# zkp-gravity/0g-halo2

Measured on AMD Instinct MI355X. Metric: create_proof proofs/hour, model_28input_256entry_1hash_1bpi, higher is better.
Workload: dtype u32x8 (254-bit Montgomery integers)

## Files before the change

### 0g-halo2_amd/csrc/field.h

```cpp
#pragma once

#include <hip/hip_runtime.h>
#include <stdint.h>

#define ZG_HD __host__ __device__ __forceinline__

namespace zg {

struct alignas(16) Fe {
    uint32_t l[8];
};

struct FrParams {
    static ZG_HD uint32_t p(int i) {
        constexpr uint32_t P[8] = {0xf0000001u, 0x43e1f593u, 0x79b97091u, 0x2833e848u,
                                   0x8181585du, 0xb85045b6u, 0xe131a029u, 0x30644e72u};
        return P[i];
    }
    static constexpr uint32_t P_TOP = 0x30644e72u;
    static constexpr uint32_t INV = 0xefffffffu;
    static constexpr bool IS_FR = true;
    static ZG_HD Fe one() {
        return Fe{{0x4ffffffbu, 0xac96341cu, 0x9f60cd29u, 0x36fc7695u, 0x7879462eu, 0x666ea36fu,
                   0x9a07df2fu, 0x0e0a77c1u}};
// ... 129 lines not shown
#include "mont_mul_gfx950.inc"
        Fe o;
#pragma unroll
        for (int i = 0; i < 8; i++) o.l[i] = r[i];
        reduce_once(o);
        return o;
#else
        typedef unsigned __int128 u128;
        uint64_t A[4], B[4], M[4], t[6] = {0, 0, 0, 0, 0, 0};
        for (int i = 0; i < 4; i++) {
            A[i] = (uint64_t)a.l[2 * i] | ((uint64_t)a.l[2 * i + 1] << 32);
            B[i] = (uint64_t)b.l[2 * i] | ((uint64_t)b.l[2 * i + 1] << 32);
            M[i] = (uint64_t)P::p(2 * i) | ((uint64_t)P::p(2 * i + 1) << 32);
        }
        const uint64_t ninv32 = P::INV;
        const uint64_t inv64 = ninv32 * (2 + M[0] * ninv32);
        for (int i = 0; i < 4; i++) {
            u128 c = 0;
            for (int j = 0; j < 4; j++) {
                c += (u128)A[j] * B[i] + t[j];
                t[j] = (uint64_t)c;
                c >>= 64;
            }
            c += t[4];
            t[4] = (uint64_t)c;
            t[5] = (uint64_t)(c >> 64);
            const uint64_t m = t[0] * inv64;
            c = (u128)m * M[0] + t[0];
            c >>= 64;
            for (int j = 1; j < 4; j++) {
                c += (u128)m * M[j] + t[j];
                t[j - 1] = (uint64_t)c;
                c >>= 64;
            }
            c += t[4];
            t[3] = (uint64_t)c;
            t[4] = t[5] + (uint64_t)(c >> 64);
        }
        Fe o;
        for (int i = 0; i < 4; i++) {
            o.l[2 * i] = (uint32_t)t[i];
            o.l[2 * i + 1] = (uint32_t)(t[i] >> 32);
        }
        reduce_once(o);
        return o;
#endif
    }

    static ZG_HD Fe sqr(const Fe& a) { return mul(a, a); }

    static ZG_HD Fe from_raw(const Fe& a) { return mul(a, P::r2()); }

    static ZG_HD Fe to_raw(const Fe& a) {
        Fe one_raw = fe_zero();
        one_raw.l[0] = 1;
        return mul(a, one_raw);
    }

    static ZG_HD Fe from_u64(uint64_t v) {
        Fe t = fe_zero();
        t.l[0] = (uint32_t)v;
        t.l[1] = (uint32_t)(v >> 32);
        return from_raw(t);
    }

    static ZG_HD Fe pow(const Fe& a, const uint32_t e[8]) {
        Fe res = one();
        for (int i = 7; i >= 0; i--)
            for (int b = 31; b >= 0; b--) {
                res = sqr(res);
                if ((e[i] >> b) & 1) res = mul(res, a);
            }
        return res;
    }

    static ZG_HD Fe pow_u64(const Fe& a, uint64_t e) {
        Fe res = one();
        bool started = false;
        for (int b = 63; b >= 0; b--) {
            if (started) res = sqr(res);
            if ((e >> b) & 1) {
                res = mul(res, a);
                started = true;
            }
        }
        return res;
    }

    static ZG_HD Fe inv_fermat(const Fe& a) {
        uint32_t e[8];
#pragma unroll
        for (int i = 0; i < 8; i++) e[i] = P::p(i);
        e[0] -= 2;
        return pow(a, e);
    }

    static ZG_HD Fe inv(const Fe& a) {
        if (fe_is_zero(a)) return a;
#if !defined(__HIP_DEVICE_COMPILE__)
        {
            typedef unsigned __int128 u128;
            uint64_t pm4[4], u[4], v[4], x1[4] = {1, 0, 0, 0}, x2[4] = {0, 0, 0, 0};
            for (int i = 0; i < 4; i++) {
                pm4[i] = (uint64_t)P::p(2 * i) | ((uint64_t)P::p(2 * i + 1) << 32);
                u[i] = (uint64_t)a.l[2 * i] | ((uint64_t)a.l[2 * i + 1] << 32);
                v[i] = pm4[i];
            }
            auto add4 = [](uint64_t* o, const uint64_t* x, const uint64_t* y) {
                u128 c = 0;
// ... 138 lines not shown
```

### 0g-halo2_amd/csrc/msm.hip

```cpp
#include <cstdlib>

#include "msm.h"
#include "field9.h"

namespace zg {

constexpr uint32_t MSM_K_THROUGHPUT = 48, MSM_K_LATENCY = 16;
constexpr uint32_t MSM_MAX_C = 16;
constexpr uint32_t MSM_LEN_BINS = 128;
constexpr uint32_t MSM_HEAVY = 16;
constexpr uint32_t MSM_HEAVY_THROUGHPUT = 4;
constexpr uint32_t MSM_AFFINE_ROUNDS = 0;
constexpr uint32_t MSM_MAX_BATCH = 4096;

__device__ __forceinline__ Fe ld_fe_g(const Fe* p) {
    Fe r;
    const uint4* q = reinterpret_cast<const uint4*>(p);
    uint4 a = q[0], b = q[1];
    r.l[0] = a.x; r.l[1] = a.y; r.l[2] = a.z; r.l[3] = a.w;
    r.l[4] = b.x; r.l[5] = b.y; r.l[6] = b.z; r.l[7] = b.w;
    return r;
}
__device__ __forceinline__ void st_fe_g(Fe* p, const Fe& v) {
    uint4* q = reinterpret_cast<uint4*>(p);
    q[0] = make_uint4(v.l[0], v.l[1], v.l[2], v.l[3]);
    q[1] = make_uint4(v.l[4], v.l[5], v.l[6], v.l[7]);
}
__device__ __forceinline__ XYZZ ld_xyzz(const XYZZ* p) {
    XYZZ r;
    r.x = ld_fe_g(&p->x); r.y = ld_fe_g(&p->y); r.zz = ld_fe_g(&p->zz); r.zzz = ld_fe_g(&p->zzz);
    return r;
}
__device__ __forceinline__ void st_xyzz(XYZZ* p, const XYZZ& v) {
    st_fe_g(&p->x, v.x); st_fe_g(&p->y, v.y); st_fe_g(&p->zz, v.zz); st_fe_g(&p->zzz, v.zzz);
}

__global__ void msm_table_kernel(const Affine* __restrict__ bases, Affine* __restrict__ table,
                                 uint32_t n, uint32_t c, uint32_t windows) {
    uint32_t i = blockIdx.x * blockDim.x + threadIdx.x;
    if (i >= n) return;
    const Fe c261 = Fq9Params::c261_fe();
    Affine p;
    p.x = ld_fe_g(&bases[i].x);
    p.y = ld_fe_g(&bases[i].y);
    st_fe_g(&table[i].x, Fq::mul(p.x, c261));
    st_fe_g(&table[i].y, Fq::mul(p.y, c261));
    for (uint32_t w = 1; w < windows; w++) {
        XYZZ acc = xyzz_dbl_affine(p);
        for (uint32_t d = 1; d < c; d++) acc = xyzz_dbl(acc);
        p = xyzz_to_affine(acc);
        st_fe_g(&table[(size_t)w * n + i].x, Fq::mul(p.x, c261));
        st_fe_g(&table[(size_t)w * n + i].y, Fq::mul(p.y, c261));
    }
}

__global__ __launch_bounds__(256) void msm_digits_kernel(const Fe* __restrict__ scalars, size_t stride, uint32_t per,
                                                         size_t outer, uint32_t n,
                                                         uint32_t c, uint32_t windows, uint32_t tbits,
                                                         uint32_t* __restrict__ dig, uint64_t run_mask) {
    uint32_t i = blockIdx.x * blockDim.x + threadIdx.x, b = blockIdx.y;
    if (i >= n) return;
    const uint32_t nb = 1u << (c - 1);
    const uint32_t j = b % per;
    const Fe* sv = scalars + (size_t)(b / per) * outer + (size_t)j * stride;
    Fe s = ld_fe_g(sv + i);
    uint32_t flip = 0;
    if (j < 64 && ((run_mask >> j) & 1ull)) {
        if (i + 1 < n) s = Fr::sub(s, ld_fe_g(sv + i + 1));
        s = Fr::to_raw(s);
        Fe neg;
        uint32_t ps[8], pr[8];
#pragma unroll
        for (int j = 0; j < 8; j++) {
            ps[j] = s.l[j];
            pr[j] = FrParams::p(j);
        }
        uint32_t nl[8];
        sub8(nl, pr, ps);
#pragma unroll
        for (int j = 0; j < 8; j++) neg.l[j] = nl[j];
        bool smaller = false;
        for (int j = 7; j >= 0; j--) {
            if (neg.l[j] != s.l[j]) {
                smaller = neg.l[j] < s.l[j];
                break;
            }
        }
        if (smaller && !fe_is_zero(s)) {
            s = neg;
            flip = 1u << 31;
        }
    } else {
        s = Fr::to_raw(s);
    }
    uint32_t l[9];
#pragma unroll
    for (int j = 0; j < 8; j++) l[j] = s.l[j];
    l[8] = 0;
    const uint32_t top_lo = c * (windows - 1) - 1;
    bool large = false;
#pragma unroll
    for (int j = 0; j < 8; j++) {
        const uint32_t lo_bit = 32u * j;
        if (lo_bit + 32 > top_lo) {
            uint32_t v = l[j];
            if (lo_bit < top_lo) v >>= (top_lo - lo_bit);
            large |= v != 0;
        }
    }
    if (large && tbits) {
        const uint32_t t = ((l[0] >> 5) ^ (l[1] >> 11) ^ l[2]) & ((1u << tbits) - 1);
        uint64_t carry = 0;
#pragma unroll
        for (int j = 0; j < 8; j++) {
            carry += (uint64_t)l[j] + (uint64_t)t * FrParams::p(j);
            l[j] = (uint32_t)carry;
            carry >>= 32;
        }
        l[8] = (uint32_t)carry;
    }
    uint64_t bits = (uint64_t)l[0] | ((uint64_t)l[1] << 32);
    uint32_t have = 64, next = 2, carry = 0;
    uint32_t* db = dig + (size_t)b * windows * n + i;
    for (uint32_t w = 0; w < windows; w++) {
        if (have < c && next < 9) {
            uint32_t limb = next == 2 ? l[2] : next == 3 ? l[3] : next == 4 ? l[4] : next == 5 ? l[5]
                          : next == 6 ? l[6] : next == 7 ? l[7] : l[8];
            bits |= (uint64_t)limb << have;
            have += 32;
            next++;
        }
        uint32_t d = (uint32_t)(bits & ((1u << c) - 1)) + carry;
        bits >>= c;
        have = have >= c ? have - c : 0;
        carry = d > nb ? 1u : 0u;
        uint32_t k = carry ? (1u << c) - d : d;
        db[(size_t)w * n] = k ? (k | ((carry << 31) ^ flip)) : 0u;
    }
}

static_assert((FrParams::P_TOP >> 30) == 0, "msm_digits_naf_kernel: the scalar field's modulus must be below 2^254");
__global__ __launch_bounds__(256) void msm_digits_naf_kernel(const Fe* __restrict__ scalars, size_t stride, uint32_t per,
                                                             size_t outer, uint32_t n, uint32_t w, uint32_t slots,
                                                             uint32_t* __restrict__ dig, uint64_t run_mask, uint32_t balanced) {
    const uint32_t i = blockIdx.x * blockDim.x + threadIdx.x, b = blockIdx.y;
    if (i >= n) return;
    const uint32_t vj = b % per;
    const Fe* sv = scalars + (size_t)(b / per) * outer + (size_t)vj * stride;
    Fe s = ld_fe_g(sv + i);
    uint32_t flip = 0;
    if (vj < 64 && ((run_mask >> vj) & 1ull)) {
        if (i + 1 < n) s = Fr::sub(s, ld_fe_g(sv + i + 1));
        s = Fr::to_raw(s);
        Fe neg, pr;
#pragma unroll
        for (int j = 0; j < 8; j++) pr.l[j] = FrParams::p(j);
        sub8(neg.l, pr.l, s.l);
        bool smaller = false;
        for (int j = 7; j >= 0; j--) {
            if (neg.l[j] != s.l[j]) {
                smaller = neg.l[j] < s.l[j];
                break;
            }
        }
        if (smaller && !fe_is_zero(s)) {
            s = neg;
            flip = 0x80000000u;
        }
    } else {
        s = Fr::to_raw(s);
    }
    uint64_t bits = (uint64_t)s.l[0];
    uint32_t have = 32, next = 1, pos = 0, slot = 0;
    uint32_t* db = dig + (size_t)b * slots * n + i;
    const uint32_t mask = (1u << w) - 1u, half = 1u << (w - 1);
    for (;;) {
        if (have <= 16 && next < 8) {
            const uint32_t limb = next == 1 ? s.l[1] : next == 2 ? s.l[2] : next == 3 ? s.l[3] : next == 4 ? s.l[4]
                                : next == 5 ? s.l[5] : next == 6 ? s.l[6] : s.l[7];
            bits += (uint64_t)limb << have;
            have += 32;
            next++;
        }
        if (bits == 0 && next >= 8) break;
        if ((bits & 1ull) == 0) {
            uint32_t z = bits ? (uint32_t)__ffsll((long long)bits) - 1u : have;
            if (z > have) z = have;
            if (z == 0) z = 1;
            bits >>= z;
            have -= z;
            pos += z;
            continue;
        }
        uint32_t wd = w, m = mask, hf = half;
        if (balanced && next >= 8) {
            const uint32_t rem = 64u - (uint32_t)__clzll((long long)bits);
            if (rem <= w - 1u) {
                if (slot < slots && pos <= 254u) db[(size_t)slot * n] = (((uint32_t)bits + 1u) >> 1) | (pos << 16) | flip;
                slot++;
                break;
            }
            if (rem <= 2u * (w - 1u)) {
                wd = (rem + 1u) >> 1;
                m = (1u << wd) - 1u;
                hf = 1u << (wd - 1u);
            }
        }
        const uint32_t v = (uint32_t)bits & m;
        const bool neg = v > hf;
        const uint32_t d = neg ? (m + 1u) - v : v;
        if (slot < slots && pos <= 254u) db[(size_t)slot * n] = ((d + 1u) >> 1) | (pos << 16) | ((neg ? 0x80000000u : 0u) ^ flip);
        slot++;
        bits = (bits >> wd) + (neg ? 1ull : 0ull);
        have = have >= wd ? have - wd : 0;
        pos += wd;
    }
    for (; slot < slots; slot++) db[(size_t)slot * n] = 0u;
}

__global__ __launch_bounds__(1024) void msm_hist_kernel(const uint32_t* __restrict__ dig, uint32_t n, uint32_t c,
                                                        uint32_t windows, uint32_t* __restrict__ cnt,
// ... 668 lines not shown
template <int L, uint32_t RB>
__global__ __launch_bounds__(L * RB) void msm_bucket_sum_kernel(const XYZZ9* __restrict__ sfx,
                                                                                   const XYZZ9* __restrict__ blk_p,
                                                                                   XYZZ9* __restrict__ blk_w,
                                                                                   uint32_t nblk, uint32_t* __restrict__ tickets,
                                                                                   XYZZ* __restrict__ out, uint32_t odd,
                                                                                   XYZZ9* __restrict__ tsum) {
    __shared__ XYZZ9 sh[RB];
    __shared__ XYZZ9 bs;
    const uint32_t j = threadIdx.x / L, role = threadIdx.x % L;
    const uint32_t blk = blockIdx.x, b = blockIdx.y;
    if (role == 0) sh[j] = blk + 1 + j < nblk ? ld_xyzz9(blk_p + (size_t)b * nblk + blk + 1 + j) : xyzz9_identity();
    __syncthreads();
    uint32_t span = 1;
    while (span < nblk) span <<= 1;
    auto tree_step = [&](uint32_t o) {
        if (j < o) xstore<true>(&sh[j], xaddl<L>(&sh[j], &sh[j + o], role));
        __syncthreads();
    };
    for (uint32_t o = span / 2; o > 0; o >>= 1) tree_step(o);
    if (threadIdx.x == 0) bs = sh[0];
    __syncthreads();
    xstore<true>(&sh[j], xaddl<L>(sfx + ((size_t)b * nblk + blk) * RB + j, &bs, role));
    __syncthreads();
    if (odd && blk == 0 && threadIdx.x == 0) st_xyzz9(tsum + b, sh[0]);
    __syncthreads();
    for (uint32_t o = RB / 2; o > 0; o >>= 1) tree_step(o);
    __shared__ uint32_t ticket;
    if (threadIdx.x == 0) {
        st_xyzz9(blk_w + (size_t)b * nblk + blk, sh[0]);
        __threadfence();
        ticket = atomicAdd(tickets + b, 1u);
    }
    __syncthreads();
    if (ticket != nblk - 1) return;
    __threadfence();
    if (role == 0) sh[j] = j < nblk ? ld_xyzz9(blk_w + (size_t)b * nblk + j) : xyzz9_identity();
    __syncthreads();
    for (uint32_t o = span / 2; o > 0; o >>= 1) tree_step(o);
    if (threadIdx.x == 0) {
        XYZZ9 R = sh[0];
        if (odd) {
            XYZZ9 T = ld_xyzz9(tsum + b);
            R = xyzz9_add(R, R);
            T.y = f9_neg(T.y);
            R = xyzz9_add(R, T);
        }
        st_xyzz(out + b, xyzz9_to_xyzz(R, false));
        tickets[b] = 0;
    }
}

constexpr uint32_t MSM_STRIP = 8;
constexpr uint32_t MSM_STRIP_LANES = 256;

__global__ __launch_bounds__(256) void msm_strip_kernel(const XYZZ9* __restrict__ partial, const uint32_t* __restrict__ toff,
                                                        const uint32_t* __restrict__ hmap, const XYZZ9* __restrict__ hsum,
                                                        uint32_t max_tasks, uint32_t max_heavy, uint32_t c, uint32_t nstrips,
                                                        XYZZ9* __restrict__ strip_u, XYZZ9* __restrict__ strip_loc, uint32_t S) {
    const uint32_t j = blockIdx.x * blockDim.x + threadIdx.x, b = blockIdx.y;
    if (j >= nstrips) return;
    const uint32_t nb = 1u << (c - 1);
    const uint32_t* to = toff + (size_t)b * (nb + 2);
    const XYZZ9* pp = partial + (size_t)b * max_tasks;
    XYZZ9 run = xyzz9_identity(), loc = xyzz9_identity();
    for (uint32_t s = S; s-- > 0;) {
        const uint32_t k = j * S + s + 1;
        if (k <= nb) {
            const uint32_t hs = hmap[(size_t)b * (nb + 1) + k];
            if (hs < max_heavy) {
                run = xyzz9_add(run, ld_xyzz9(hsum + (size_t)b * max_heavy + hs));
            } else {
                const uint32_t t0 = to[k], t1 = to[k + 1];
                for (uint32_t t = t0; t < t1; t++) run = xyzz9_add(run, ld_xyzz9(pp + t));
            }
        }
        loc = xyzz9_add(loc, run);
    }
    st_xyzz9(strip_u + (size_t)b * nstrips + j, run);
    st_xyzz9(strip_loc + (size_t)b * nstrips + j, loc);
}

__global__ __launch_bounds__(MSM_STRIP_LANES) void msm_strip_sum_kernel(const XYZZ9* __restrict__ strip_u,
                                                                       const XYZZ9* __restrict__ strip_loc, uint32_t nstrips,
                                                                       uint32_t per, XYZZ* __restrict__ out, uint32_t S, uint32_t odd) {
    __shared__ XYZZ9 sh[MSM_STRIP_LANES];
    const uint32_t l = threadIdx.x, b = blockIdx.x;
    const XYZZ9* U = strip_u + (size_t)b * nstrips;
    const XYZZ9* L = strip_loc + (size_t)b * nstrips;
    XYZZ9 C = xyzz9_identity(), w = xyzz9_identity(), a = xyzz9_identity();
    for (uint32_t t = per; t-- > 0;) {
        const uint32_t jj = l * per + t;
        if (jj >= nstrips) continue;
        w = xyzz9_add(w, C);
        C = xyzz9_add(C, ld_xyzz9(U + jj));
        a = xyzz9_add(a, ld_xyzz9(L + jj));
    }
    auto tree = [&](XYZZ9 v) {
        sh[l] = v;
        __syncthreads();
        for (uint32_t o = MSM_STRIP_LANES / 2; o > 0; o >>= 1) {
            if (l < o) sh[l] = xyzz9_add(sh[l], sh[l + o]);
            __syncthreads();
        }
        XYZZ9 r = sh[0];
        __syncthreads();
        return r;
    };
    sh[l] = C;
    __syncthreads();
    for (uint32_t o = 1; o < MSM_STRIP_LANES; o <<= 1) {
        XYZZ9 v = xyzz9_identity();
        const bool has = l + o < MSM_STRIP_LANES;
        if (has) v = sh[l + o];
        __syncthreads();
        if (has) sh[l] = xyzz9_add(sh[l], v);
        __syncthreads();
    }
    XYZZ9 sfx = l >= 1 ? sh[l] : xyzz9_identity();
    __syncthreads();
    XYZZ9 X = sfx;
    for (uint32_t d = per; d > 1; d >>= 1) X = xyzz9_dbl(X);
    X = xyzz9_add(X, w);
    for (uint32_t d = S; d > 1; d >>= 1) X = xyzz9_dbl(X);
    XYZZ9 Y = xyzz9_add(X, a);
    if (odd) {
        Y = xyzz9_dbl(Y);
        XYZZ9 nc = C;
        nc.y = f9_neg(nc.y);
        Y = xyzz9_add(Y, nc);
    }
    const XYZZ9 R = tree(Y);
    if (l != 0) return;
    st_xyzz(out + b, xyzz9_to_xyzz(R, false));
}

static uint32_t default_window_bits(size_t n) {
    if (const int v = knob(K_MSM_C); v >= 2 && v <= (int)MSM_MAX_C) return (uint32_t)v;
    uint32_t lg = 0;
    while (((size_t)1 << (lg + 1)) <= n) lg++;
    int c = lg >= 14 ? (int)lg - 2 : (int)lg - 1;
    if (c < 4) c = 4;
    if (c > (int)MSM_MAX_C) c = MSM_MAX_C;
    return (uint32_t)c;
}

int bases_register_dev(zg_ctx* ctx, const Affine* d_bases, size_t n, uint32_t window_bits, zg_bases** out) {
    ZG_REQUIRE(n > 0 && n < (1u << 23), ZG_ERR_UNSUPPORTED, "zg_bases_register: n=%zu out of range", n);
    uint32_t c = window_bits ? window_bits : default_window_bits(n);
    ZG_REQUIRE(c >= 1 && c <= MSM_MAX_C, ZG_ERR_INVALID_ARG, "zg_bases_register: window_bits %u not in [2,16]", c);
    uint32_t windows = (255 + c - 1) / c;
    zg_bases* b = new zg_bases();
    b->ctx = ctx;
    b->device = ctx->device;
    b->n = n;
    b->c = c;
    b->windows = windows;
    hipError_t e = hipMalloc(&b->table, (size_t)windows * n * sizeof(Affine));
    if (e != hipSuccess) {
        set_error("zg_bases_register: hipMalloc(%zu) failed: %s", (size_t)windows * n * sizeof(Affine),
                  hipGetErrorString(e));
        delete b;
        return ZG_ERR_OOM;
    }
    hipLaunchKernelGGL(msm_table_kernel, dim3((uint32_t)((n + 63) / 64)), dim3(64), 0, ctx->stream, d_bases,
                       b->table, (uint32_t)n, c, windows);
// ... 475 lines not shown
    uint32_t R;
    size_t cap;
    uint64_t left;
    uint32_t max_tasks;
    bool pair_tasks;
    uint32_t rb, nblk;
    int lanes;
    uint32_t heavy_thr, max_heavy;
    uint32_t strip, nstrips, strip_per;
    uint32_t tbits;
    uint32_t topsplit;
};
static int msm_plan(const zg_ctx* ctx, const MsmJob& j, uint32_t naf, MsmPlan* out) {
    MsmPlan p{};
    const size_t n = j.n;
    p.B = (uint32_t)j.batch; p.N = (uint32_t)n; p.naf = naf;
    p.c = naf ? naf - 1 : j.bases->c; p.W = naf ? 254 / naf + 1 : j.bases->windows; p.nb = 1u << (p.c - 1);
    const int k_env = knob(K_MSM_K);
    const int kl_env = knob(K_MSM_K_LAT);
    const uint32_t k_lat_default = n >= (1u << 17) ? 48u : n >= (1u << 16) ? 32u : MSM_K_LATENCY;
    p.K = ctx->msm_pair ? (kl_env >= 4 && kl_env <= 120 ? (uint32_t)kl_env : k_lat_default)
                        : (k_env >= 4 && k_env <= 120 ? (uint32_t)k_env : MSM_K_THROUGHPUT);
    p.entries = (uint64_t)p.N * p.W;
    ZG_REQUIRE(p.entries < (1ull << 31), ZG_ERR_UNSUPPORTED, "zg_msm: n*windows too large");
    const int aff_env = knob(K_MSM_AFFINE);
    p.R = ctx->msm_pair ? 0u : aff_env >= 0 && aff_env <= 4 ? (uint32_t)aff_env : MSM_AFFINE_ROUNDS;
    const uint64_t padm = (1ull << p.R) - 1ull;
    p.cap = (size_t)((p.entries + (uint64_t)p.nb * padm + padm) & ~padm);
    ZG_REQUIRE(p.cap < (1ull << 31), ZG_ERR_UNSUPPORTED, "zg_msm: n*windows too large");
    p.left = p.cap >> p.R;
    p.max_tasks = (uint32_t)(p.left / p.K + (p.left < p.nb ? p.left : p.nb) + 1);
    p.pair_tasks = ctx->msm_pair && p.N < (1u << 16);
    p.rb = MSM_RB;
    p.lanes = 1;
    if (ctx->msm_pair) {
        const int rb_env = knob(K_MSM_RB), lanes_env = knob(K_MSM_LANES);
        const uint32_t nblk64 = (p.nb + 63) / 64;
        const bool quad_fits = nblk64 <= 64 && (uint64_t)nblk64 * p.B <= (uint64_t)ctx->num_cus;
        uint32_t want = rb_env == 64 || rb_env == 128 || rb_env == 256 ? (uint32_t)rb_env : quad_fits ? 64u : 128u;
        if ((p.nb + want - 1) / want <= want) p.rb = want;
        p.lanes = lanes_env == 2 || lanes_env == 4 ? lanes_env : p.rb == 64 ? 4 : 2;
        if (p.rb > 128) p.lanes = 2;
    }
    p.nblk = (p.nb + p.rb - 1) / p.rb;
    ZG_REQUIRE(p.nblk <= 256 && p.nblk <= p.rb, ZG_ERR_UNSUPPORTED, "zg_msm: window_bits %u too large", p.c);
    const int hv_env = knob(K_MSM_HEAVY);
    p.heavy_thr = hv_env >= 1 && hv_env <= 64 ? (uint32_t)hv_env : ctx->msm_pair ? MSM_HEAVY : MSM_HEAVY_THROUGHPUT;
    p.max_heavy = (uint32_t)(p.left / ((uint64_t)p.heavy_thr * p.K)) + 1;
    if (p.max_heavy > p.nb) p.max_heavy = p.nb;
    const int s_env = knob(K_MSM_STRIP);
    p.strip = s_env == 2 || s_env == 4 || s_env == 8 || s_env == 16 ? (uint32_t)s_env : MSM_STRIP;
    p.nstrips = (p.nb + p.strip - 1) / p.strip;
    p.strip_per = 1;
    while (p.strip_per * MSM_STRIP_LANES < p.nstrips) p.strip_per <<= 1;
    const int spare = (int)(p.c * p.W) - 1 - 254;
    if (spare >= 1) p.tbits = (uint32_t)spare;
    if (p.tbits > 10) p.tbits = 10;
    p.topsplit = knob(K_MSM_TOPSPLIT) != 0 ? 1u : 0u;
    *out = p;
    return ZG_OK;
}

struct MsmWs {
    uint32_t *dig, *cnt, *slot, *off, *toff, *tot, *ttotal, *stoff, *sbucket, *sorted;
    XYZZ9* partial;
    Affine *pts_odd, *pts_even;
    int32_t *aff_pre, *aff_val, *aff_pfx, *aff_val2, *aff_pfx2;
    XYZZ9 *blk_w, *tsum, *blk_p, *sfx;
    uint32_t *hmap, *hlist, *nheavy;
    XYZZ9* hsum;
};
static bool msm_workspace(WsScope& ws, const MsmPlan& p, MsmWs* out) {
    const uint32_t B = p.B, W = p.W, nb = p.nb, R = p.R;
    const size_t cap = p.cap;
    MsmWs w{};
    w.dig = ws.get<uint32_t>((size_t)B * p.entries);
    w.cnt = ws.get<uint32_t>((size_t)B * W * (nb + 1));
    w.slot = ws.get<uint32_t>((size_t)B * p.entries);
    w.off = ws.get<uint32_t>((size_t)B * W * (nb + 1));
    w.toff = ws.get<uint32_t>((size_t)B * (nb + 2));
    w.tot = ws.get<uint32_t>((size_t)B * (nb + 2));
    w.ttotal = ws.get<uint32_t>(B);
    w.stoff = ws.get<uint32_t>((size_t)B * (nb + 2));
    w.sbucket = ws.get<uint32_t>((size_t)B * (nb + 1));
    w.sorted = ws.get<uint32_t>((size_t)B * cap);
    w.partial = ws.get<XYZZ9>((size_t)B * p.max_tasks);
    const uint32_t aff_lanes = R ? (uint32_t)((((cap >> 1) + AFF_A - 1) / AFF_A + 255) / 256 * 256) : 0u;
    const size_t aff_n1 = (size_t)B * aff_lanes, aff_n2 = (aff_n1 + AFF_S - 1) / AFF_S;
    w.pts_odd = R >= 1 ? ws.get<Affine>((size_t)B * (cap >> 1)) : nullptr;
    w.pts_even = R >= 2 ? ws.get<Affine>((size_t)B * (cap >> 2)) : nullptr;
    w.aff_pre = R ? ws.get<int32_t>((size_t)9 * AFF_A * aff_n1) : nullptr;
    w.aff_val = R ? ws.get<int32_t>((size_t)9 * aff_n1) : nullptr;
    w.aff_pfx = R ? ws.get<int32_t>((size_t)9 * aff_n1) : nullptr;
    w.aff_val2 = R ? ws.get<int32_t>((size_t)9 * aff_n2) : nullptr;
    w.aff_pfx2 = R ? ws.get<int32_t>((size_t)9 * aff_n2) : nullptr;
    w.blk_w = ws.get<XYZZ9>((size_t)B * p.nblk);
    w.tsum = ws.get<XYZZ9>(B);
    w.blk_p = ws.get<XYZZ9>((size_t)B * p.nblk);
    w.sfx = ws.get<XYZZ9>((size_t)B * p.nblk * p.rb);
    w.hmap = ws.get<uint32_t>((size_t)B * (nb + 1));
    w.hlist = ws.get<uint32_t>((size_t)B * p.max_heavy);
    w.nheavy = ws.get<uint32_t>(B);
    w.hsum = ws.get<XYZZ9>((size_t)B * p.max_heavy);
    *out = w;
    return !ws.failed;
}

// ... 41 lines not shown
                  w.aff_pfx, n1, w.aff_val2, n2);
        ZG_LAUNCH(ctx, "msm_aff_invert", (double)n2 * 108.0, aff_inv_top_kernel, dim3(1), dim3(AFF_TOP), 0, w.aff_val2, w.aff_pfx2, n2);
        ZG_LAUNCH(ctx, "msm_aff_invert", (double)n1 * 108.0, aff_inv_down_kernel, dim3((uint32_t)((n2 + 255) / 256)), dim3(256), 0, w.aff_val,
                  w.aff_pfx, n1, w.aff_val2, n2);
        if (r == 1) ZG_LAUNCH(ctx, "msm_aff_apply", pr * (8.0 + 128.0 + 36.0 + 64.0), aff_apply_kernel<true>, g, dim3(256), 0, a);
        else ZG_LAUNCH(ctx, "msm_aff_apply", pr * (128.0 + 36.0 + 64.0), aff_apply_kernel<false>, g, dim3(256), 0, a);
        aff_pts = a.out;
    }
    return aff_pts;
}

static void msm_launch_accumulate(zg_ctx* ctx, const MsmJob& j, const MsmPlan& p, const MsmWs& w, const Affine* aff_pts) {
    const MsmTables t = msm_tables(j);
    const double msm_bytes = (double)p.B * ((double)p.N * 96.0 + 96.0);
    using AccKernel = decltype(&msm_accumulate_kernel<false, false>);
    const AccKernel acc = p.pair_tasks ? &msm_accumulate_kernel<true, false>
                          : p.R        ? &msm_accumulate_kernel<false, true>
                                       : &msm_accumulate_kernel<false, false>;
    const uint32_t lanes = p.pair_tasks ? 2 * p.max_tasks : p.max_tasks;
    ZG_LAUNCH_U(ctx, "msm_accumulate", msm_bytes, msm_bytes, acc, dim3((lanes + 255) / 256, p.B), dim3(256), 0, t.a, t.b,
                (uint32_t)j.split, (uint32_t)j.bases->n, p.c, p.W, p.N, w.tot, w.toff, w.ttotal, w.sorted, p.max_tasks, w.partial, t.run_a,
                t.run_b, j.run_mask, (uint32_t)j.per, w.stoff, w.sbucket, p.cap, p.pair_tasks ? 0u : p.R, p.pair_tasks ? nullptr : aff_pts);
}

static void msm_launch_reduce(zg_ctx* ctx, const MsmJob& j, const MsmPlan& p, const MsmWs& w) {
    const uint32_t B = p.B, c = p.c, nb = p.nb, nblk = p.nblk, max_tasks = p.max_tasks, max_heavy = p.max_heavy;
    const double part_bytes = (double)B * (double)(nb < max_tasks ? nb : max_tasks) * sizeof(XYZZ9);
    const dim3 hgrid(MSM_HEAVY_WGS);
    if (ctx->msm_pair) {
        ZG_LAUNCH(ctx, "msm_heavy", (double)B * 4.0, msm_heavy_kernel<2>, hgrid, dim3(512), 0, w.partial, w.toff, w.hlist, w.nheavy, max_tasks,
                  max_heavy, c, w.hsum, B);
        auto reduce = [&](auto ltag, auto rtag) {
            constexpr int L = decltype(ltag)::value;
            constexpr uint32_t RB = decltype(rtag)::value;
            ZG_LAUNCH(ctx, "msm_bucket_scan", part_bytes + (double)B * nblk * (RB + 1.0) * sizeof(XYZZ9), (msm_bucket_scan_kernel<L, RB>), dim3(nblk, B), dim3(L * RB), 0,
                      w.partial, w.toff, w.hmap, w.hsum, max_tasks, max_heavy, c, w.sfx, w.blk_p, nblk);
            ZG_LAUNCH(ctx, "msm_bucket_sum", (double)B * nblk * (RB + 2.0) * sizeof(XYZZ9), (msm_bucket_sum_kernel<L, RB>), dim3(nblk, B), dim3(L * RB), 0, w.sfx,
                      w.blk_p, w.blk_w, nblk, ctx->msm_tickets, j.out, p.naf ? 1u : 0u, w.tsum);
        };
        using I2 = std::integral_constant<int, 2>;
        using I4 = std::integral_constant<int, 4>;
        if (p.rb == 64 && p.lanes == 4) reduce(I4{}, std::integral_constant<uint32_t, 64>{});
        else if (p.rb == 64) reduce(I2{}, std::integral_constant<uint32_t, 64>{});
        else if (p.rb == 128 && p.lanes == 4) reduce(I4{}, std::integral_constant<uint32_t, 128>{});
        else if (p.rb == 128) reduce(I2{}, std::integral_constant<uint32_t, 128>{});
        else reduce(I2{}, std::integral_constant<uint32_t, MSM_RB>{});
    } else {
        ZG_LAUNCH(ctx, "msm_heavy", (double)B * 4.0, msm_heavy_groups_kernel, hgrid, dim3(256), 0, w.partial, w.toff, w.hlist, w.nheavy,
                  max_tasks, max_heavy, c, w.hsum, B);
        const uint32_t nstrips = p.nstrips;
        XYZZ9 *strip_u = w.sfx, *strip_loc = w.sfx + (size_t)B * nstrips;
        ZG_LAUNCH(ctx, "msm_strip", part_bytes + (double)B * 2.0 * nstrips * sizeof(XYZZ9), msm_strip_kernel, dim3((nstrips + 255) / 256, B), dim3(256), 0, w.partial,
                  w.toff, w.hmap, w.hsum, max_tasks, max_heavy, c, nstrips, strip_u, strip_loc, p.strip);
        ZG_LAUNCH(ctx, "msm_strip_sum", (double)B * (2.0 * nstrips * sizeof(XYZZ9) + sizeof(XYZZ)), msm_strip_sum_kernel, dim3(B), dim3(MSM_STRIP_LANES), 0, strip_u, strip_loc,
                  nstrips, p.strip_per, j.out, p.strip, p.naf ? 1u : 0u);
    }
}

int msm_dev(zg_ctx* ctx, const MsmJob& job) {
    MsmJob j = job;
    uint32_t naf = 0;
    ZG_TRY(msm_check(j, &naf));
    if (j.batch == 0) return ZG_OK;
    if (j.n == 0) {
        std::vector<XYZZ> ids(j.batch, xyzz_identity());
        ZG_HIP(hipMemcpyAsync(j.out, ids.data(), j.batch * sizeof(XYZZ), hipMemcpyDefault, ctx->stream));
        ZG_HIP(hipStreamSynchronize(ctx->stream));
        return ZG_OK;
    }
    if (msm_full_applies(ctx, j, naf)) return msm_full_dev(ctx, j);
    MsmPlan plan;
    ZG_TRY(msm_plan(ctx, j, naf, &plan));
    if (!ctx->msm_tickets) {
        gate_yield(ctx);
        ZG_HIP(hipMalloc(&ctx->msm_tickets, MSM_MAX_BATCH * sizeof(uint32_t)));
        ZG_HIP(hipMemset(ctx->msm_tickets, 0, MSM_MAX_BATCH * sizeof(uint32_t)));
    }
    ZG_REQUIRE(plan.B <= MSM_MAX_BATCH, ZG_ERR_UNSUPPORTED, "zg_msm: batch of %u vectors", (unsigned)plan.B);
    WsScope ws(ctx);
    MsmWs w;
    if (!msm_workspace(ws, plan, &w)) return ZG_ERR_OOM;
    {
        DeviceState& ds = device_state(ctx->device);
        std::lock_guard<std::mutex> lock(ds.mu);
        if (!ds.msm_attrs) {
            ZG_HIP(hipFuncSetAttribute((const void*)msm_hist_kernel, hipFuncAttributeMaxDynamicSharedMemorySize, 160 * 1024));
            ZG_HIP(hipFuncSetAttribute((const void*)msm_scan_kernel, hipFuncAttributeMaxDynamicSharedMemorySize, 150 * 1024));
            ds.msm_attrs = true;
        }
    }
    msm_launch_sort(ctx, j, plan, w);
    msm_launch_accumulate(ctx, j, plan, w, msm_launch_affine(ctx, j, plan, w));
    msm_launch_reduce(ctx, j, plan, w);
    ZG_HIP(hipGetLastError());
    return ZG_OK;
}

static int msm_plain_dev(zg_ctx* ctx, const zg_bases* bases, const Fe* d_scalars, size_t stride, size_t batch, size_t n, XYZZ* d_out) {
    if (const zg_bases* d = bases_dense(bases); d && d->naf_w && !ctx->msm_pair) bases = d;
    MsmJob j;
    j.bases = bases; j.split = batch;
    j.scalars = d_scalars; j.stride = stride;
    j.batch = batch; j.n = n;
    j.out = d_out;
    return msm_dev(ctx, j);
}

// ... 157 lines not shown
```

Baseline: 5.477 million.

## Specialize Montgomery to_raw, simplify signed-digit abs, shrink strip-sum lanes

Replaces the generic multiply-by-one used for leaving Montgomery form with a dedicated reduction: inline gfx950 assembly on device and an 8-round REDC on host, which skips the partial products against zero limbs. Replaces the limb-by-limb magnitude comparison in both digit kernels with a single subtract-against-(p/2) borrow test. Also reduces the strip-sum block size to 64 or 128 lanes depending on strip count, giving shorter tree reductions and less shared memory but more sequential work per lane. The hand-written carry chain in assembly is a correctness risk.

```diff
diff --git a/0g-halo2_amd/csrc/field.h b/0g-halo2_amd/csrc/field.h
--- a/0g-halo2_amd/csrc/field.h
+++ b/0g-halo2_amd/csrc/field.h
@@ -205,9 +205,38 @@
     static ZG_HD Fe from_raw(const Fe& a) { return mul(a, P::r2()); }
 
     static ZG_HD Fe to_raw(const Fe& a) {
-        Fe one_raw = fe_zero();
-        one_raw.l[0] = 1;
-        return mul(a, one_raw);
+#if defined(__HIP_DEVICE_COMPILE__)
+        uint64_t acc = 0;
+        uint32_t ovf = 0;
+        uint32_t m[8], r[8];
+#include "mont_redc_gfx950.inc"
+        Fe o;
+#pragma unroll
+        for (int i = 0; i < 8; i++) o.l[i] = r[i];
+        reduce_once(o);
+        return o;
+#else
+        uint32_t t[8];
+#pragma unroll
+        for (int i = 0; i < 8; i++) t[i] = a.l[i];
+#pragma unroll
+        for (int i = 0; i < 8; i++) {
+            const uint32_t m = t[0] * P::INV;
+            uint64_t c = ((uint64_t)m * P::p(0) + t[0]) >> 32;
+#pragma unroll
+            for (int j = 1; j < 8; j++) {
+                c += (uint64_t)m * P::p(j) + t[j];
+                t[j - 1] = (uint32_t)c;
+                c >>= 32;
+            }
+            t[7] = (uint32_t)c;
+        }
+        Fe o;
+#pragma unroll
+        for (int i = 0; i < 8; i++) o.l[i] = t[i];
+        reduce_once(o);
+        return o;
+#endif
     }
 
     static ZG_HD Fe from_u64(uint64_t v) {
diff --git a/0g-halo2_amd/csrc/mont_redc_gfx950.inc b/0g-halo2_amd/csrc/mont_redc_gfx950.inc
--- /dev/null
+++ b/0g-halo2_amd/csrc/mont_redc_gfx950.inc
@@ -0,0 +1,54 @@
+        asm("v_mad_u64_u32 %0, vcc, %2, %3, %0\n\tv_addc_co_u32 %1, vcc, 0, 0, vcc" : "+v"(acc), "=&v"(ovf) : "v"(a.l[0]), "s"(1u) : "vcc");
+        m[0] = (uint32_t)acc * P::INV;
+        asm("v_mad_u64_u32 %0, vcc, %2, %3, %0\n\tv_addc_co_u32 %1, vcc, 0, %1, vcc" : "+v"(acc), "+v"(ovf) : "v"(m[0]), "s"(P::p(0)) : "vcc");
+        acc = (acc >> 32) | ((uint64_t)ovf << 32);
+        asm("v_mad_u64_u32 %0, vcc, %2, %3, %0\n\tv_addc_co_u32 %1, vcc, 0, 0, vcc\n\tv_mad_u64_u32 %0, vcc, %4, %5, %0\n\tv_addc_co_u32 %1, vcc, 0, %1, vcc" : "+v"(acc), "=&v"(ovf) : "v"(a.l[1]), "s"(1u), "v"(m[0]), "s"(P::p(1)) : "vcc");
+        m[1] = (uint32_t)acc * P::INV;
+        asm("v_mad_u64_u32 %0, vcc, %2, %3, %0\n\tv_addc_co_u32 %1, vcc, 0, %1, vcc" : "+v"(acc), "+v"(ovf) : "v"(m[1]), "s"(P::p(0)) : "vcc");
+        acc = (acc >> 32) | ((uint64_t)ovf << 32);
+        asm("v_mad_u64_u32 %0, vcc, %2, %3, %0\n\tv_addc_co_u32 %1, vcc, 0, 0, vcc\n\tv_mad_u64_u32 %0, vcc, %4, %5, %0\n\tv_addc_co_u32 %1, vcc, 0, %1, vcc\n\tv_mad_u64_u32 %0, vcc, %6, %7, %0\n\tv_addc_co_u32 %1, vcc, 0, %1, vcc" : "+v"(acc), "=&v"(ovf) : "v"(a.l[2]), "s"(1u), "v"(m[0]), "s"(P::p(2)), "v"(m[1]), "s"(P::p(1)) : "vcc");
+        m[2] = (uint32_t)acc * P::INV;
+        asm("v_mad_u64_u32 %0, vcc, %2, %3, %0\n\tv_addc_co_u32 %1, vcc, 0, %1, vcc" : "+v"(acc), "+v"(ovf) : "v"(m[2]), "s"(P::p(0)) : "vcc");
+        acc = (acc >> 32) | ((uint64_t)ovf << 32);
+        asm("v_mad_u64_u32 %0, vcc, %2, %3, %0\n\tv_addc_co_u32 %1, vcc, 0, 0, vcc\n\tv_mad_u64_u32 %0, vcc, %4, %5, %0\n\tv_addc_co_u32 %1, vcc, 0, %1, vcc\n\tv_mad_u64_u32 %0, vcc, %6, %7, %0\n\tv_addc_co_u32 %1, vcc, 0, %1, vcc\n\tv_mad_u64_u32 %0, vcc, %8, %9, %0\n\tv_addc_co_u32 %1, vcc, 0, %1, vcc" : "+v"(acc), "=&v"(ovf) : "v"(a.l[3]), "s"(1u), "v"(m[0]), "s"(P::p(3)), "v"(m[1]), "s"(P::p(2)), "v"(m[2]), "s"(P::p(1)) : "vcc");
+        m[3] = (uint32_t)acc * P::INV;
+        asm("v_mad_u64_u32 %0, vcc, %2, %3, %0\n\tv_addc_co_u32 %1, vcc, 0, %1, vcc" : "+v"(acc), "+v"(ovf) : "v"(m[3]), "s"(P::p(0)) : "vcc");
+        acc = (acc >> 32) | ((uint64_t)ovf << 32);
+        asm("v_mad_u64_u32 %0, vcc, %2, %3, %0\n\tv_addc_co_u32 %1, vcc, 0, 0, vcc\n\tv_mad_u64_u32 %0, vcc, %4, %5, %0\n\tv_addc_co_u32 %1, vcc, 0, %1, vcc\n\tv_mad_u64_u32 %0, vcc, %6, %7, %0\n\tv_addc_co_u32 %1, vcc, 0, %1, vcc\n\tv_mad_u64_u32 %0, vcc, %8, %9, %0\n\tv_addc_co_u32 %1, vcc, 0, %1, vcc\n\tv_mad_u64_u32 %0, vcc, %10, %11, %0\n\tv_addc_co_u32 %1, vcc, 0, %1, vcc" : "+v"(acc), "=&v"(ovf) : "v"(a.l[4]), "s"(1u), "v"(m[0]), "s"(P::p(4)), "v"(m[1]), "s"(P::p(3)), "v"(m[2]), "s"(P::p(2)), "v"(m[3]), "s"(P::p(1)) : "vcc");
+        m[4] = (uint32_t)acc * P::INV;
+        asm("v_mad_u64_u32 %0, vcc, %2, %3, %0\n\tv_addc_co_u32 %1, vcc, 0, %1, vcc" : "+v"(acc), "+v"(ovf) : "v"(m[4]), "s"(P::p(0)) : "vcc");
+        acc = (acc >> 32) | ((uint64_t)ovf << 32);
+        asm("v_mad_u64_u32 %0, vcc, %2, %3, %0\n\tv_addc_co_u32 %1, vcc, 0, 0, vcc\n\tv_mad_u64_u32 %0, vcc, %4, %5, %0\n\tv_addc_co_u32 %1, vcc, 0, %1, vcc\n\tv_mad_u64_u32 %0, vcc, %6, %7, %0\n\tv_addc_co_u32 %1, vcc, 0, %1, vcc\n\tv_mad_u64_u32 %0, vcc, %8, %9, %0\n\tv_addc_co_u32 %1, vcc, 0, %1, vcc\n\tv_mad_u64_u32 %0, vcc, %10, %11, %0\n\tv_addc_co_u32 %1, vcc, 0, %1, vcc\n\tv_mad_u64_u32 %0, vcc, %12, %13, %0\n\tv_addc_co_u32 %1, vcc, 0, %1, vcc" : "+v"(acc), "=&v"(ovf) : "v"(a.l[5]), "s"(1u), "v"(m[0]), "s"(P::p(5)), "v"(m[1]), "s"(P::p(4)), "v"(m[2]), "s"(P::p(3)), "v"(m[3]), "s"(P::p(2)), "v"(m[4]), "s"(P::p(1)) : "vcc");
+        m[5] = (uint32_t)acc * P::INV;
+        asm("v_mad_u64_u32 %0, vcc, %2, %3, %0\n\tv_addc_co_u32 %1, vcc, 0, %1, vcc" : "+v"(acc), "+v"(ovf) : "v"(m[5]), "s"(P::p(0)) : "vcc");
+        acc = (acc >> 32) | ((uint64_t)ovf << 32);
+        asm("v_mad_u64_u32 %0, vcc, %2, %3, %0\n\tv_addc_co_u32 %1, vcc, 0, 0, vcc\n\tv_mad_u64_u32 %0, vcc, %4, %5, %0\n\tv_addc_co_u32 %1, vcc, 0, %1, vcc\n\tv_mad_u64_u32 %0, vcc, %6, %7, %0\n\tv_addc_co_u32 %1, vcc, 0, %1, vcc\n\tv_mad_u64_u32 %0, vcc, %8, %9, %0\n\tv_addc_co_u32 %1, vcc, 0, %1, vcc\n\tv_mad_u64_u32 %0, vcc, %10, %11, %0\n\tv_addc_co_u32 %1, vcc, 0, %1, vcc\n\tv_mad_u64_u32 %0, vcc, %12, %13, %0\n\tv_addc_co_u32 %1, vcc, 0, %1, vcc\n\tv_mad_u64_u32 %0, vcc, %14, %15, %0\n\tv_addc_co_u32 %1, vcc, 0, %1, vcc" : "+v"(acc), "=&v"(ovf) : "v"(a.l[6]), "s"(1u), "v"(m[0]), "s"(P::p(6)), "v"(m[1]), "s"(P::p(5)), "v"(m[2]), "s"(P::p(4)), "v"(m[3]), "s"(P::p(3)), "v"(m[4]), "s"(P::p(2)), "v"(m[5]), "s"(P::p(1)) : "vcc");
+        m[6] = (uint32_t)acc * P::INV;
+        asm("v_mad_u64_u32 %0, vcc, %2, %3, %0\n\tv_addc_co_u32 %1, vcc, 0, %1, vcc" : "+v"(acc), "+v"(ovf) : "v"(m[6]), "s"(P::p(0)) : "vcc");
+        acc = (acc >> 32) | ((uint64_t)ovf << 32);
+        asm("v_mad_u64_u32 %0, vcc, %2, %3, %0\n\tv_addc_co_u32 %1, vcc, 0, 0, vcc\n\tv_mad_u64_u32 %0, vcc, %4, %5, %0\n\tv_addc_co_u32 %1, vcc, 0, %1, vcc\n\tv_mad_u64_u32 %0, vcc, %6, %7, %0\n\tv_addc_co_u32 %1, vcc, 0, %1, vcc\n\tv_mad_u64_u32 %0, vcc, %8, %9, %0\n\tv_addc_co_u32 %1, vcc, 0, %1, vcc\n\tv_mad_u64_u32 %0, vcc, %10, %11, %0\n\tv_addc_co_u32 %1, vcc, 0, %1, vcc\n\tv_mad_u64_u32 %0, vcc, %12, %13, %0\n\tv_addc_co_u32 %1, vcc, 0, %1, vcc\n\tv_mad_u64_u32 %0, vcc, %14, %15, %0\n\tv_addc_co_u32 %1, vcc, 0, %1, vcc\n\tv_mad_u64_u32 %0, vcc, %16, %17, %0\n\tv_addc_co_u32 %1, vcc, 0, %1, vcc" : "+v"(acc), "=&v"(ovf) : "v"(a.l[7]), "s"(1u), "v"(m[0]), "s"(P::p(7)), "v"(m[1]), "s"(P::p(6)), "v"(m[2]), "s"(P::p(5)), "v"(m[3]), "s"(P::p(4)), "v"(m[4]), "s"(P::p(3)), "v"(m[5]), "s"(P::p(2)), "v"(m[6]), "s"(P::p(1)) : "vcc");
+        m[7] = (uint32_t)acc * P::INV;
+        asm("v_mad_u64_u32 %0, vcc, %2, %3, %0\n\tv_addc_co_u32 %1, vcc, 0, %1, vcc" : "+v"(acc), "+v"(ovf) : "v"(m[7]), "s"(P::p(0)) : "vcc");
+        acc = (acc >> 32) | ((uint64_t)ovf << 32);
+        asm("v_mad_u64_u32 %0, vcc, %2, %3, %0\n\tv_addc_co_u32 %1, vcc, 0, 0, vcc\n\tv_mad_u64_u32 %0, vcc, %4, %5, %0\n\tv_addc_co_u32 %1, vcc, 0, %1, vcc\n\tv_mad_u64_u32 %0, vcc, %6, %7, %0\n\tv_addc_co_u32 %1, vcc, 0, %1, vcc\n\tv_mad_u64_u32 %0, vcc, %8, %9, %0\n\tv_addc_co_u32 %1, vcc, 0, %1, vcc\n\tv_mad_u64_u32 %0, vcc, %10, %11, %0\n\tv_addc_co_u32 %1, vcc, 0, %1, vcc\n\tv_mad_u64_u32 %0, vcc, %12, %13, %0\n\tv_addc_co_u32 %1, vcc, 0, %1, vcc\n\tv_mad_u64_u32 %0, vcc, %14, %15, %0\n\tv_addc_co_u32 %1, vcc, 0, %1, vcc" : "+v"(acc), "=&v"(ovf) : "v"(m[1]), "s"(P::p(7)), "v"(m[2]), "s"(P::p(6)), "v"(m[3]), "s"(P::p(5)), "v"(m[4]), "s"(P::p(4)), "v"(m[5]), "s"(P::p(3)), "v"(m[6]), "s"(P::p(2)), "v"(m[7]), "s"(P::p(1)) : "vcc");
+        r[0] = (uint32_t)acc;
+        acc = (acc >> 32) | ((uint64_t)ovf << 32);
+        asm("v_mad_u64_u32 %0, vcc, %2, %3, %0\n\tv_addc_co_u32 %1, vcc, 0, 0, vcc\n\tv_mad_u64_u32 %0, vcc, %4, %5, %0\n\tv_addc_co_u32 %1, vcc, 0, %1, vcc\n\tv_mad_u64_u32 %0, vcc, %6, %7, %0\n\tv_addc_co_u32 %1, vcc, 0, %1, vcc\n\tv_mad_u64_u32 %0, vcc, %8, %9, %0\n\tv_addc_co_u32 %1, vcc, 0, %1, vcc\n\tv_mad_u64_u32 %0, vcc, %10, %11, %0\n\tv_addc_co_u32 %1, vcc, 0, %1, vcc\n\tv_mad_u64_u32 %0, vcc, %12, %13, %0\n\tv_addc_co_u32 %1, vcc, 0, %1, vcc" : "+v"(acc), "=&v"(ovf) : "v"(m[2]), "s"(P::p(7)), "v"(m[3]), "s"(P::p(6)), "v"(m[4]), "s"(P::p(5)), "v"(m[5]), "s"(P::p(4)), "v"(m[6]), "s"(P::p(3)), "v"(m[7]), "s"(P::p(2)) : "vcc");
+        r[1] = (uint32_t)acc;
+        acc = (acc >> 32) | ((uint64_t)ovf << 32);
+        asm("v_mad_u64_u32 %0, vcc, %2, %3, %0\n\tv_addc_co_u32 %1, vcc, 0, 0, vcc\n\tv_mad_u64_u32 %0, vcc, %4, %5, %0\n\tv_addc_co_u32 %1, vcc, 0, %1, vcc\n\tv_mad_u64_u32 %0, vcc, %6, %7, %0\n\tv_addc_co_u32 %1, vcc, 0, %1, vcc\n\tv_mad_u64_u32 %0, vcc, %8, %9, %0\n\tv_addc_co_u32 %1, vcc, 0, %1, vcc\n\tv_mad_u64_u32 %0, vcc, %10, %11, %0\n\tv_addc_co_u32 %1, vcc, 0, %1, vcc" : "+v"(acc), "=&v"(ovf) : "v"(m[3]), "s"(P::p(7)), "v"(m[4]), "s"(P::p(6)), "v"(m[5]), "s"(P::p(5)), "v"(m[6]), "s"(P::p(4)), "v"(m[7]), "s"(P::p(3)) : "vcc");
+        r[2] = (uint32_t)acc;
+        acc = (acc >> 32) | ((uint64_t)ovf << 32);
+        asm("v_mad_u64_u32 %0, vcc, %2, %3, %0\n\tv_addc_co_u32 %1, vcc, 0, 0, vcc\n\tv_mad_u64_u32 %0, vcc, %4, %5, %0\n\tv_addc_co_u32 %1, vcc, 0, %1, vcc\n\tv_mad_u64_u32 %0, vcc, %6, %7, %0\n\tv_addc_co_u32 %1, vcc, 0, %1, vcc\n\tv_mad_u64_u32 %0, vcc, %8, %9, %0\n\tv_addc_co_u32 %1, vcc, 0, %1, vcc" : "+v"(acc), "=&v"(ovf) : "v"(m[4]), "s"(P::p(7)), "v"(m[5]), "s"(P::p(6)), "v"(m[6]), "s"(P::p(5)), "v"(m[7]), "s"(P::p(4)) : "vcc");
+        r[3] = (uint32_t)acc;
+        acc = (acc >> 32) | ((uint64_t)ovf << 32);
+        asm("v_mad_u64_u32 %0, vcc, %2, %3, %0\n\tv_addc_co_u32 %1, vcc, 0, 0, vcc\n\tv_mad_u64_u32 %0, vcc, %4, %5, %0\n\tv_addc_co_u32 %1, vcc, 0, %1, vcc\n\tv_mad_u64_u32 %0, vcc, %6, %7, %0\n\tv_addc_co_u32 %1, vcc, 0, %1, vcc" : "+v"(acc), "=&v"(ovf) : "v"(m[5]), "s"(P::p(7)), "v"(m[6]), "s"(P::p(6)), "v"(m[7]), "s"(P::p(5)) : "vcc");
+        r[4] = (uint32_t)acc;
+        acc = (acc >> 32) | ((uint64_t)ovf << 32);
+        asm("v_mad_u64_u32 %0, vcc, %2, %3, %0\n\tv_addc_co_u32 %1, vcc, 0, 0, vcc\n\tv_mad_u64_u32 %0, vcc, %4, %5, %0\n\tv_addc_co_u32 %1, vcc, 0, %1, vcc" : "+v"(acc), "=&v"(ovf) : "v"(m[6]), "s"(P::p(7)), "v"(m[7]), "s"(P::p(6)) : "vcc");
+        r[5] = (uint32_t)acc;
+        acc = (acc >> 32) | ((uint64_t)ovf << 32);
+        asm("v_mad_u64_u32 %0, vcc, %2, %3, %0\n\tv_addc_co_u32 %1, vcc, 0, 0, vcc" : "+v"(acc), "=&v"(ovf) : "v"(m[7]), "s"(P::p(7)) : "vcc");
+        r[6] = (uint32_t)acc;
+        acc = (acc >> 32) | ((uint64_t)ovf << 32);
+        r[7] = (uint32_t)acc;
diff --git a/0g-halo2_amd/csrc/msm.hip b/0g-halo2_amd/csrc/msm.hip
--- a/0g-halo2_amd/csrc/msm.hip
+++ b/0g-halo2_amd/csrc/msm.hip
@@ -54,6 +54,21 @@
     }
 }
 
+__device__ __forceinline__ Fe run_form_abs(const Fe& s, uint32_t& flip) {
+    uint32_t pr[8], hf[8], t[8];
+#pragma unroll
+    for (int j = 0; j < 8; j++) {
+        pr[j] = FrParams::p(j);
+        hf[j] = FrParams::p(j) >> 1;
+        if (j < 7) hf[j] |= FrParams::p(j + 1) << 31;
+    }
+    Fe neg;
+    sub8(neg.l, pr, s.l);
+    if (!sub8(t, hf, s.l)) return s;
+    flip = 0x80000000u;
+    return neg;
+}
+
 __global__ __launch_bounds__(256) void msm_digits_kernel(const Fe* __restrict__ scalars, size_t stride, uint32_t per,
                                                          size_t outer, uint32_t n,
                                                          uint32_t c, uint32_t windows, uint32_t tbits,
@@ -67,29 +82,7 @@
     uint32_t flip = 0;
     if (j < 64 && ((run_mask >> j) & 1ull)) {
         if (i + 1 < n) s = Fr::sub(s, ld_fe_g(sv + i + 1));
-        s = Fr::to_raw(s);
-        Fe neg;
-        uint32_t ps[8], pr[8];
-#pragma unroll
-        for (int j = 0; j < 8; j++) {
-            ps[j] = s.l[j];
-            pr[j] = FrParams::p(j);
-        }
-        uint32_t nl[8];
-        sub8(nl, pr, ps);
-#pragma unroll
-        for (int j = 0; j < 8; j++) neg.l[j] = nl[j];
-        bool smaller = false;
-        for (int j = 7; j >= 0; j--) {
-            if (neg.l[j] != s.l[j]) {
-                smaller = neg.l[j] < s.l[j];
-                break;
-            }
-        }
-        if (smaller && !fe_is_zero(s)) {
-            s = neg;
-            flip = 1u << 31;
-        }
+        s = run_form_abs(Fr::to_raw(s), flip);
     } else {
         s = Fr::to_raw(s);
     }
@@ -151,22 +144,7 @@
     uint32_t flip = 0;
     if (vj < 64 && ((run_mask >> vj) & 1ull)) {
         if (i + 1 < n) s = Fr::sub(s, ld_fe_g(sv + i + 1));
-        s = Fr::to_raw(s);
-        Fe neg, pr;
-#pragma unroll
-        for (int j = 0; j < 8; j++) pr.l[j] = FrParams::p(j);
-        sub8(neg.l, pr.l, s.l);
-        bool smaller = false;
-        for (int j = 7; j >= 0; j--) {
-            if (neg.l[j] != s.l[j]) {
-                smaller = neg.l[j] < s.l[j];
-                break;
-            }
-        }
-        if (smaller && !fe_is_zero(s)) {
-            s = neg;
-            flip = 0x80000000u;
-        }
+        s = run_form_abs(Fr::to_raw(s), flip);
     } else {
         s = Fr::to_raw(s);
     }
@@ -941,7 +919,8 @@
 }
 
 constexpr uint32_t MSM_STRIP = 8;
-constexpr uint32_t MSM_STRIP_LANES = 256;
+constexpr uint32_t MSM_STRIP_LANES = 128;
+static uint32_t msm_strip_lanes(uint32_t nstrips) { return nstrips <= 256 ? 64u : MSM_STRIP_LANES; }
 
 __global__ __launch_bounds__(256) void msm_strip_kernel(const XYZZ9* __restrict__ partial, const uint32_t* __restrict__ toff,
                                                         const uint32_t* __restrict__ hmap, const XYZZ9* __restrict__ hsum,
@@ -974,7 +953,7 @@
                                                                        const XYZZ9* __restrict__ strip_loc, uint32_t nstrips,
                                                                        uint32_t per, XYZZ* __restrict__ out, uint32_t S, uint32_t odd) {
     __shared__ XYZZ9 sh[MSM_STRIP_LANES];
-    const uint32_t l = threadIdx.x, b = blockIdx.x;
+    const uint32_t l = threadIdx.x, b = blockIdx.x, lanes = blockDim.x;
     const XYZZ9* U = strip_u + (size_t)b * nstrips;
     const XYZZ9* L = strip_loc + (size_t)b * nstrips;
     XYZZ9 C = xyzz9_identity(), w = xyzz9_identity(), a = xyzz9_identity();
@@ -988,7 +967,7 @@
     auto tree = [&](XYZZ9 v) {
         sh[l] = v;
         __syncthreads();
-        for (uint32_t o = MSM_STRIP_LANES / 2; o > 0; o >>= 1) {
+        for (uint32_t o = lanes / 2; o > 0; o >>= 1) {
             if (l < o) sh[l] = xyzz9_add(sh[l], sh[l + o]);
             __syncthreads();
         }
@@ -998,9 +977,9 @@
     };
     sh[l] = C;
     __syncthreads();
-    for (uint32_t o = 1; o < MSM_STRIP_LANES; o <<= 1) {
+    for (uint32_t o = 1; o < lanes; o <<= 1) {
         XYZZ9 v = xyzz9_identity();
-        const bool has = l + o < MSM_STRIP_LANES;
+        const bool has = l + o < lanes;
         if (has) v = sh[l + o];
         __syncthreads();
         if (has) sh[l] = xyzz9_add(sh[l], v);
@@ -1582,7 +1561,7 @@
     p.strip = s_env == 2 || s_env == 4 || s_env == 8 || s_env == 16 ? (uint32_t)s_env : MSM_STRIP;
     p.nstrips = (p.nb + p.strip - 1) / p.strip;
     p.strip_per = 1;
-    while (p.strip_per * MSM_STRIP_LANES < p.nstrips) p.strip_per <<= 1;
+    while (p.strip_per * msm_strip_lanes(p.nstrips) < p.nstrips) p.strip_per <<= 1;
     const int spare = (int)(p.c * p.W) - 1 - 254;
     if (spare >= 1) p.tbits = (uint32_t)spare;
     if (p.tbits > 10) p.tbits = 10;
@@ -1730,7 +1709,7 @@
         XYZZ9 *strip_u = w.sfx, *strip_loc = w.sfx + (size_t)B * nstrips;
         ZG_LAUNCH(ctx, "msm_strip", part_bytes + (double)B * 2.0 * nstrips * sizeof(XYZZ9), msm_strip_kernel, dim3((nstrips + 255) / 256, B), dim3(256), 0, w.partial,
                   w.toff, w.hmap, w.hsum, max_tasks, max_heavy, c, nstrips, strip_u, strip_loc, p.strip);
-        ZG_LAUNCH(ctx, "msm_strip_sum", (double)B * (2.0 * nstrips * sizeof(XYZZ9) + sizeof(XYZZ)), msm_strip_sum_kernel, dim3(B), dim3(MSM_STRIP_LANES), 0, strip_u, strip_loc,
+        ZG_LAUNCH(ctx, "msm_strip_sum", (double)B * (2.0 * nstrips * sizeof(XYZZ9) + sizeof(XYZZ)), msm_strip_sum_kernel, dim3(B), dim3(msm_strip_lanes(nstrips)), 0, strip_u, strip_loc,
                   nstrips, p.strip_per, j.out, p.strip, p.naf ? 1u : 0u);
     }
 }
```

Result: no change. 5.520 million, median of 6 (+0.8%).
